# hidasib/GRU4Rec

Measured on AMD Instinct MI355X. Metric: mini-batches/sec (gru4rec.py:661), RSC15-shaped batch=128 n_sample=2048 BPR-max, higher is better.
Workload: dtype f32

## Files before the change

### gru4rec_amd/csrc/g4r_eval_kernels.cuh

```cuda
#pragma once
#include "g4r_step_kernels.cuh"

#define SC_BM 128
#define SC_KC 128

template <int TN, bool COUNT = false>
__global__ __launch_bounds__(256) void k_score_all(const DevModel* __restrict__ mp, const float* h, int mrows, const int* item_idx,
                                                   long long n_sel, float* out, long long ldo, int apply_act,
                                                   int* cnt = nullptr, long long col_begin = 0, const int* tie_col = nullptr,
                                                   unsigned tie_ctr = 0) {
    extern __shared__ __attribute__((aligned(16))) float smem[];
    const DevModel& m = *mp;
    const int tid = threadIdx.x, lane = tid & 63, wid = tid >> 6, li = lane & 15, lg = lane >> 4;
    const int D = m.Dtop;
    const int ldk = SC_KC + 2;
    float* sA = smem;
    float* sB = sA + SC_BM * ldk;
    int* sItem = reinterpret_cast<int*>(sB + TN * ldk);
    const long long n0 = (long long)blockIdx.x * TN;
    const int rbase = blockIdx.y * SC_BM;
    if (tid < TN) {
        const long long n = n0 + tid;
        int item = -1;
        if (n < n_sel) item = item_idx ? item_idx[n] : (int)n;
// ... 182 lines not shown

__global__ void k_selftest_mfma32(const float* A, const float* Bm, float* C, int K) {
    const int lane = threadIdx.x & 63, l32 = lane & 31, lh = lane >> 5;
    f32x16 acc;
    for (int j = 0; j < 16; ++j) acc[j] = 0.f;
    for (int k = 0; k < K; k += 2) acc = mfma32(A[l32 * K + k + lh], Bm[(k + lh) * 32 + l32], acc);
    for (int r = 0; r < 16; ++r) C[(8 * (r >> 2) + 4 * lh + (r & 3)) * 32 + l32] = acc[r];
}

template __global__ void k_sparse_update<1, false>(const DevModel*, StepState*, int);
template __global__ void k_sparse_update<1, true>(const DevModel*, StepState*, int);
template __global__ void k_sparse_update<2, false>(const DevModel*, StepState*, int);
template __global__ void k_sparse_update<2, true>(const DevModel*, StepState*, int);
template __global__ void k_sparse_update_generic<1>(const DevModel*, StepState*, int, int);
template __global__ void k_sparse_update_generic<2>(const DevModel*, StepState*, int, int);
template __global__ void k_loss_rows<false, 0, 1>(const DevModel*, StepState*);
template __global__ void k_loss_rows<false, 0, 4>(const DevModel*, StepState*);
template __global__ void k_loss_rows<false, 1, 1>(const DevModel*, StepState*);
template __global__ void k_loss_rows<false, 1, 4>(const DevModel*, StepState*);
template __global__ void k_loss_rows<false, 2, 1>(const DevModel*, StepState*);
template __global__ void k_loss_rows<false, 2, 4>(const DevModel*, StepState*);
template __global__ void k_loss_rows<false, 3, 1>(const DevModel*, StepState*);
template __global__ void k_loss_rows<false, 3, 4>(const DevModel*, StepState*);
template __global__ void k_loss_rows<true, 0, 4>(const DevModel*, StepState*);
template __global__ void k_loss_rows<true, 1, 4>(const DevModel*, StepState*);
template __global__ void k_loss_rows<true, 2, 4>(const DevModel*, StepState*);
template __global__ void k_loss_rows<true, 3, 4>(const DevModel*, StepState*);
template __global__ void k_sparse_update<4, false>(const DevModel*, StepState*, int);
template __global__ void k_sparse_update<4, true>(const DevModel*, StepState*, int);
template __global__ void k_sparse_update_generic<4>(const DevModel*, StepState*, int, int);
template __global__ void k_update<1, 32, false>(const DevModel*, StepState*, const DenseTile*, int, int);
template __global__ void k_update<1, 32, true>(const DevModel*, StepState*, const DenseTile*, int, int);
template __global__ void k_update<2, 32, false>(const DevModel*, StepState*, const DenseTile*, int, int);
template __global__ void k_update<2, 32, true>(const DevModel*, StepState*, const DenseTile*, int, int);
template __global__ void k_dense_grad<32>(const DevModel*, StepState*, const DenseTile*);
template __global__ void k_score_fwd<GT_BN, GT_BK>(const DevModel*, StepState*);
template __global__ void k_score_fwd<32, 64>(const DevModel*, StepState*);
template __global__ void k_score_fwd<64, 32, T2_BK>(const DevModel*, StepState*);
template __global__ void k_score_fwd<64, 32, 3>(const DevModel*, StepState*);
template __global__ void k_score_bwd<32, GT_BK>(const DevModel*, StepState*, int, int, int, int);
template __global__ void k_score_bwd<64, 64>(const DevModel*, StepState*, int, int, int, int);
template __global__ void k_gru_p1<GT_BN, P1_BK>(const DevModel*, StepState*, int, int, int, GruFwdPredict);
// ... 8 lines not shown
```

### gru4rec_amd/csrc/g4r_host_create.hpp

```cpp

int g4r_device_count(void) {
    int n = 0;
    if (hipGetDeviceCount(&n) != hipSuccess) return 0;
    return n;
}
const char* g4r_last_error(void) { return g_err.c_str(); }
#ifndef G4R_HIPCC_VERSION
#define G4R_HIPCC_VERSION "unknown"
#endif
const char* g4r_version(void) { return "gru4rec_hip 0.4 (gfx950; hipcc " G4R_HIPCC_VERSION "; isa-audited)"; }
int g4r_sizeof_config(void) { return (int)sizeof(g4r_config); }

static int build_lean_args(g4r_model* m) {
    DevModel& d = m->dm;
    const StepKernels& k = m->kern;
    const int L = d.n_layers;
    std::vector<LeanV> av(L); std::vector<LeanH> ah(L); std::vector<LeanDa> aa(L); std::vector<LeanDy> ay(L);
    const bool constrained = d.embed_mode == G4R_EMBED_CONSTRAINED;
    bool any_layer = false;
    for (int l = 0; l < L; ++l) {
        if (k.fwd[l] != FWD_LEAN) continue;
        any_layer = true;
        LeanV& v = av[l]; memset(&v, 0, sizeof(v));
        v.Wx = d.dense_p + d.offWx[l]; v.Wrz = d.dense_p + d.offWrz[l]; v.Bh = d.dense_p + d.offBh[l];
// ... 59 lines not shown
        m->h_leanU.own_on = d.own_pos ? 1 : 0;
        const bool pays = cdiv(d.R, LOSS_NW) > G4R_OWN_WINDOW_MINWG;
        m->own_window = d.own_pos && d.R <= G4R_OWN_WINDOW_MAXR && (m->sw.owner_window > 0 || (m->sw.owner_window < 0 && pays));
        HIPCHK(hipMemcpyAsync(m->d_tiles16, tiles.data(), tiles.size() * sizeof(DenseTile), hipMemcpyHostToDevice, m->stream));
        HIPCHK(hipStreamSynchronize(m->stream));
    }
    HIPCHK(hipStreamSynchronize(m->stream));
    return 0;
}

static KernelSwitches read_switches(const g4r_config& cfg) {
    KernelSwitches w;
    w.no_lean = getenv("G4R_NO_LEAN") != nullptr; w.no_mt = getenv("G4R_NO_MT") != nullptr; w.no_bmt = getenv("G4R_NO_BMT") != nullptr;
    w.no_merge = getenv("G4R_NO_MERGE") != nullptr; w.owner_scan_in_update = env_int("G4R_OWNER_SCAN", 0) != 0;
    w.owner_window = env_int("G4R_OWNER_WINDOW", -1);
    w.score_b_split = env_int("G4R_SCORE_B_SPLIT", 1) != 0;
    w.allow_lean_update = env_int("G4R_LEAN_UPDATE", 1) != 0; w.defer = env_int("G4R_DEFER", cfg.defer_updates) != 0;
    w.p2_geo = env_int("G4R_P2_GEO", -1); w.ba_geo = env_int("G4R_BA_GEO", -1);
    w.wide2 = env_int("G4R_WIDE2", -1); w.p1_ks = env_int("G4R_P1_KS", 128); w.bb_ks = env_int("G4R_BB_KS", 0);
    const char* skip = getenv("G4R_SKIP_KN");
    w.skip_kn = skip ? strtoull(skip, nullptr, 0) : 0ull;
    return w;
}

int g4r_create(const g4r_config* cfg, g4r_model** out) {
    if (!cfg || !out) return fail("null argument");
    if (cfg->n_layers < 1 || cfg->n_layers > G4R_MAX_LAYERS) return fail("n_layers out of range");
    if (cfg->batch_size < 1 || cfg->n_items < 1) return fail("batch_size / n_items must be positive");
    for (int l = 0; l < cfg->n_layers; ++l)
        if (cfg->layers[l] % 4 != 0 || cfg->layers[l] < 4 || cfg->layers[l] > 1024)
// ... 275 lines not shown
```

### gru4rec_amd/csrc/g4r_host_debug.hpp

```cpp
int g4r_get_debug(g4r_model* m, const char* name, float* host, int64_t count) {
    if (!m || !name || !host) return fail("null argument");
    HIPCHK(hipSetDevice(m->cfg.device));
    DevModel& d = m->dm;
    const StepKernels& k = m->kern;
    std::string s(name);
    const float* p = nullptr; int64_t n = 0;
    int l = 0;
    if (!s.empty() && isdigit((unsigned char)s.back())) { l = s.back() - '0'; s.pop_back(); }
    if (l >= d.n_layers) return fail("layer out of range");
    const int64_t bd = (int64_t)d.B * d.D[l];
    if (s == "scores") { p = d.Sc; n = (int64_t)d.B * d.ldSc; }
    else if (s == "dSx") { p = d.dSx + (size_t)((m->gstep - 1) & d.defer_mask) * (size_t)d.dSx_stride; n = (int64_t)d.B * d.Ein; }
    else if (s == "dSy") { p = d.dSy + (size_t)((m->gstep - 1) & d.defer_mask) * (size_t)d.dSy_stride; n = (int64_t)d.ldSc * d.Dtop; }
    else if (s == "dSBy") { p = d.dSBy + (size_t)((m->gstep - 1) & d.defer_mask) * (size_t)d.dSBy_stride; n = d.ldSc; }
    else if (s == "defer_stats") {
        if (count < 4) return fail("count");
        double rows = 0, bias = 0;
        if (m->defer_on) {
            std::vector<unsigned> st(2048);
            HIPCHK(hipStreamSynchronize(m->stream));
            HIPCHK(hipMemcpy(st.data(), d.dstat, st.size() * sizeof(unsigned), hipMemcpyDeviceToHost));
            for (size_t i = 0; i < st.size(); i += 2) { rows += st[i]; bias += st[i + 1]; }
        }
        host[0] = (float)rows; host[1] = (float)bias; host[2] = m->defer_on ? 1.f : 0.f; host[3] = (float)(d.defer_mask + 1);
// ... 25 lines not shown
    else if (s == "hd") { p = d.hd[l]; n = bd; }
    else if (s == "r") { p = d.r[l]; n = bd; }
    else if (s == "z") { p = d.z[l]; n = bd; }
    else if (s == "c") { p = d.c[l]; n = bd; }
    else if (s == "Hr") { p = d.Hr[l]; n = bd; }
    else if (s == "dV") { p = d.dV[l]; n = bd * 3; }
    else if (s == "dyl") { p = d.dyl[l]; n = bd; }
    else if (s == "Hprev") { p = d.H[l][(m->gstep + 1) & 1]; n = bd; }
    else if (s == "occ_idx") { p = (const float*)d.occ_idx; n = d.R; }
    else if (s == "own_pos") {
        if (!d.own_pos) return fail("no owner table (k_update_l not chosen, or G4R_OWNER_SCAN=1)");
        p = (const float*)(d.own_pos + (m->own_window ? (size_t)m->own_last * d.R * 16 : (size_t)0)); n = 16 * (int64_t)d.R;
    }
    else if (s == "own_pos_ring") { if (!d.own_pos) return fail("no owner table (k_update_l not chosen, or G4R_OWNER_SCAN=1)"); p = (const float*)d.own_pos; n = (int64_t)G4R_OWN_SLOTS * 16 * d.R; }
    else if (s == "owner_window") { if (count < 1) return fail("count"); host[0] = (m->own_window && k.update == UP_LEAN) ? 1.f : 0.f; return 0; }
#if !defined(G4R_CLK_TRACE)
    else if (s == "dbgclk" || s == "dbgtile") return fail("in-kernel traces need a library built with G4R_BUILD_CLK=1 (python -m gru4rec_amd.build --force) and G4R_CLK=1 at run time");
#endif
    else if (s == "dbgclk") { if (!d.dbgclk) return fail("G4R_CLK not set"); p = (const float*)d.dbgclk; n = 2 * (64 + 8 * (int64_t)d.R); }
    else if (s == "dbgtile") { if (!d.dbgtile) return fail("G4R_CLK not set"); p = (const float*)d.dbgtile; n = 2 * 8 * (int64_t)8192; }
    else if (s == "ntiles") { if (count < 1) return fail("count"); host[0] = (float)m->ntiles; return 0; }
    else if (s == "ldSc") { if (count < 1) return fail("count"); host[0] = (float)d.ldSc; return 0; }
    else if (s == "wide_mask") {
        if (count < 1) return fail("count");
        int mk = k.wide_dense ? 16 : 0;
        for (int l = 0; l < d.n_layers; ++l) mk |= k.wg[l].use;
        host[0] = (float)mk; return 0;
    }
    else if (s == "deep_geo") {
        if (count < 1) return fail("count");
// ... 48 lines not shown
}

int g4r_debug_loss_rows(g4r_model* m, float* scores, int64_t count, int32_t M, float* lossrow) {
    if (!m || !scores || !lossrow) return fail("null argument");
    DevModel& d = m->dm;
    if (count != (int64_t)d.B * d.ldSc) return fail("size mismatch for the score rows: expected " + std::to_string((int64_t)d.B * d.ldSc));
    if (M < 1 || M > d.B) return fail("M outside [1, batch_size]");
    HIPCHK(hipSetDevice(m->cfg.device));
    HIPCHK(hipStreamSynchronize(m->stream));
    StepState saved, mine;
    HIPCHK(hipMemcpy(&saved, (const void*)d.st, sizeof(saved), hipMemcpyDeviceToHost));
    HIPCHK(hipMemcpy((void*)d.Sc, scores, (size_t)count * sizeof(float), hipMemcpyHostToDevice));
    mine = saved;
    mine.M_b = M;
    HIPCHK(hipMemcpy((void*)d.st, &mine, sizeof(mine), hipMemcpyHostToDevice));
    launch_loss_rows(m, dim3(d.B), false, nullptr, nullptr);
    hipError_t e = hipGetLastError();
    if (e == hipSuccess) e = hipStreamSynchronize(m->stream);
    const hipError_t r = hipMemcpy((void*)d.st, &saved, sizeof(saved), hipMemcpyHostToDevice);
    if (e != hipSuccess) return fail(std::string("k_loss_rows: ") + hipGetErrorString(e));
    if (r != hipSuccess) return fail(std::string("step state: ") + hipGetErrorString(r));
    HIPCHK(hipMemcpy(scores, (const void*)d.Sc, (size_t)count * sizeof(float), hipMemcpyDeviceToHost));
    HIPCHK(hipMemcpy(lossrow, (const void*)d.lossrow, (size_t)d.B * sizeof(float), hipMemcpyDeviceToHost));
    return 0;
}

int g4r_debug_gumbel(g4r_model* m, uint64_t seed, uint32_t row_id, uint32_t step, const int32_t* items, int64_t n, float* out) {
    if (!m || !items || !out) return fail("null argument");
    if (n < 1) return fail("n must be positive");
    for (int64_t p = 0; p < n; ++p)
        if (items[p] < 0) return fail("item index out of range");
// ... 135 lines not shown
```

### gru4rec_amd/csrc/g4r_host_model.hpp

```cpp
static thread_local std::string g_err;
static int fail(const std::string& s) { g_err = s; return -1; }
void g4r_set_error(const char* fmt, ...) {
    char buf[1024];
    va_list ap;
    va_start(ap, fmt);
    vsnprintf(buf, sizeof(buf), fmt, ap);
    va_end(ap);
    g_err = buf;
}
#define HIPCHK(x)                                                                                        \
    do {                                                                                                 \
        hipError_t e_ = (x);                                                                             \
        if (e_ != hipSuccess)                                                                            \
            return fail(std::string(#x) + ": " + hipGetErrorString(e_) + " @" + std::to_string(__LINE__)); \
    } while (0)
#define NCCLCHK(x)                                                                                         \
    do {                                                                                                   \
        ncclResult_t e_ = (x);                                                                             \
        if (e_ != ncclSuccess)                                                                             \
            return fail(std::string(#x) + ": " + ncclGetErrorString(e_) + " @" + std::to_string(__LINE__)); \
    } while (0)

enum { KN_GRU_P1 = 0, KN_GRU_P2, KN_SCORE_FWD, KN_LOSS, KN_SCORE_BWD, KN_BWD_PRE, KN_BWD_A, KN_BWD_B, KN_DENSE, KN_ALLREDUCE,
       KN_DENSE_APPLY, KN_SPARSE, KN_UPDATE, KN_BWD_FUSED, KN_FWD_FUSED, KN_GATE, KN_FLUSH, KN_SCAN, KN_FINISH, KN_GRU_V, KN_GRU_H, KN_GRU_DA, KN_GRU_DY, KN_OWNER_WINDOW, KN_COUNT };
static const char* KN_NAMES[KN_COUNT] = {"k_gru_p1", "k_gru_p2", "k_score_fwd", "k_loss_rows", "k_score_bwd", "k_gru_bwd_pre",
                                         "k_gru_bwd_a", "k_gru_bwd_b", "k_dense_grad", "rccl_allreduce", "k_dense_apply",
                                         "k_sparse_update", "k_update", "k_gru_bwd", "k_gru_fwd", "k_gru_gate", "k_sparse_flush", "k_defer_scan", "k_finish_rows", "k_gru_v", "k_gru_h", "k_gru_da", "k_gru_dy", "k_owner_window"};

struct EvRec { int kn; hipEvent_t a, b; };

struct KernelSwitches {
    bool no_lean = false;
    bool no_mt = false, no_bmt = false;
    bool no_merge = false;
    bool allow_lean_update = true;
    bool score_b_split = true;
    bool owner_scan_in_update = false;
    int owner_window = -1;
    bool defer = false;
    int p2_geo = -1, ba_geo = -1;
    int wide2 = -1, p1_ks = 128, bb_ks = 0;
    unsigned long long skip_kn = 0;
};
enum GruFwdKind { FWD_LEAN = 0 , FWD_FUSED = 1 , FWD_P1S = 2 ,
                  FWD_P1_N64 = 3, FWD_P1_N32 = 4 };
enum GruBwdKind { BWD_LEAN = 0 , BWD_FUSED = 1 , BWD_ONEHOT = 2, BWD_BW = 3, BWD_B = 4 };
enum ScoreFwdKind { SF_LEAN = 0 , SF_MT = 1 , SF_T3 = 2, SF_T2 = 3, SF_K64 = 4, SF_K128 = 5  };
enum ScoreBwdKind { SB_LEAN = 0 , SB_BMT = 1 , SB_BWD2 = 2 , SB_W = 3, SB_N = 4  };
enum UpdateKind { UP_LEAN = 0 , UP_MERGED = 1 , UP_SPLIT = 2 };
struct WideGeo { int use = 0, ny = 1, nh = 1, kys = 0, khs = 0, bbn = 1, bbk = 0; };
struct StepKernels {
    int fwd[G4R_MAX_LAYERS], bwd[G4R_MAX_LAYERS];
    int p2_deep[G4R_MAX_LAYERS], ba_deep[G4R_MAX_LAYERS];
    WideGeo wg[G4R_MAX_LAYERS];
    int score_fwd;
    int loss_spec, loss_long, loss_quads;
    int score_bwd;
    int score_a_host;
    int kch, ksplit;
    int bmt_slabs;
    int nblkA, nblkB, ndtA, ndtB, nrtB;
    int update;
    int chunks;
    int wide_dense;
    int finish_rows;
};

template <class T>
struct DevBuf {
    T* p = nullptr;
    int64_t cap = 0;
    int reserve(g4r_model* m, int64_t n);
};

struct g4r_model {
    g4r_config cfg;
    DevModel dm;
// ... 320 lines not shown
            const double waste = (std::ceil(rounds) - rounds) / std::ceil(rounds) + 1e-3 * std::abs(ks - 17);
            if (waste < best) { best = waste; k.kch = kch; }
        }
    }
    k.ksplit = cdiv(d.ldSc, k.kch);
    const int TB = wide ? 64 : 32;
    k.ndtA = cdiv(Dt + 1, TB); k.nblkA = cdiv(d.ldSc, TB) * k.ndtA;
    k.ndtB = cdiv(Dt, TB); k.nrtB = cdiv(B, TB); k.nblkB = k.ksplit * k.nrtB * k.ndtB;
    const int w = std::max(Dt, d.Ein);
    k.chunks = w <= 256 ? 1 : (w <= 512 ? 2 : 4);
    const bool dy0_parts = (k.wg[0].use & 8) != 0;
    const bool merged = !d.generic && !sw.no_merge && k.chunks <= 2 && !k.wide_dense;
    const bool lean_u = !sw.no_lean && sw.allow_lean_update && merged && d.apply_dense_inplace && B <= 128 && k.chunks == 1 && !defer_on && d.xmode == 0 &&
                        !d.touched && !dy0_parts && d.R < 65536 && cdiv(d.R, 8) < 65536 && dense_tiles(d, 16, 64).size() < 65536;
    k.update = lean_u ? UP_LEAN : merged ? UP_MERGED : UP_SPLIT;
    k.finish_rows = dy0_parts && !k.wide_dense;
    return k;
}
static int sync_dm(g4r_model* m) {
    HIPCHK(hipMemcpyAsync(m->d_dm, &m->dm, sizeof(DevModel), hipMemcpyHostToDevice, m->stream));
    HIPCHK(hipStreamSynchronize(m->stream));
    return 0;
}
```

### gru4rec_amd/csrc/g4r_host_step.hpp

```cpp
static void launch_loss_rows(g4r_model* m, dim3 grid, bool timed, hipEvent_t ev_a, hipEvent_t ev_b) {
    const StepKernels& k = m->kern;
    const DevModel* dmp = (const DevModel*)m->d_dm;
    StepState* stp = (StepState*)m->dm.st;
#define G4R_LK_LOSS1(kern)                                                                                            \
    do {                                                                                                              \
        if (timed) hipExtLaunchKernelGGL(kern, grid, dim3(LOSS_T), m->smem_loss, m->stream, ev_a, ev_b, 0, dmp, stp); \
        else hipLaunchKernelGGL(kern, grid, dim3(LOSS_T), m->smem_loss, m->stream, dmp, stp);                         \
    } while (0)
#define G4R_LK_LOSS(L, V)                                                      \
    do {                                                                       \
        if (k.loss_spec == 1) G4R_LK_LOSS1((k_loss_rows<L, 1, V>));            \
        else if (k.loss_spec == 2) G4R_LK_LOSS1((k_loss_rows<L, 2, V>));       \
        else if (k.loss_spec == 3) G4R_LK_LOSS1((k_loss_rows<L, 3, V>));       \
        else G4R_LK_LOSS1((k_loss_rows<L, 0, V>));                             \
    } while (0)
    if (k.loss_long) G4R_LK_LOSS(true, 4);
    else { if (k.loss_quads) G4R_LK_LOSS(false, 4); else G4R_LK_LOSS(false, 1); }
#undef G4R_LK_LOSS
#undef G4R_LK_LOSS1
}

static int launch_step(g4r_model* m, std::vector<EvRec>* recs, int part = 0, int slot = 0) {
    DevModel& d = m->dm;
    const StepKernels& k = m->kern;
    const int L = d.n_layers, B = d.B;
    hipStream_t s = m->stream;
    GruFwdPredict nopa = {};
    size_t evi = 0;
    hipEvent_t cur_a = nullptr, cur_b = nullptr;
    static const bool trace = getenv("G4R_TRACE") != nullptr;
    int trace_kn = -1;
    auto begin = [&](int kn) {
        trace_kn = kn;
        if (trace) { fprintf(stderr, "[g4r] launch %s\n", KN_NAMES[kn]); fflush(stderr); }
        if (!recs) return;
        while (m->evs.size() < evi + 2) { hipEvent_t e; (void)hipEventCreate(&e); m->evs.push_back(e); }
        EvRec r = {kn, m->evs[evi], m->evs[evi + 1]};
// ... 77 lines not shown
                (const float*)d.Wy, (const float*)d.By, (float*)d.Sc, dimsA, dimsB);
        break;
    }
    case SF_MT: LK(k_score_mt_4s, dim3(cdiv(B, 64) * cdiv(d.ldSc, 272)), dim3(256), SMEM_MT_4S, s, (const int*)d.cur_col, (const int*)(d.cur_in + 2 * B),
                   (const float*)d.hd[L - 1], (const float*)d.Wy, (const float*)d.zrow, dmp, (unsigned)d.Dtop | ((unsigned)cdiv(B, 64) << 16),
                   (unsigned)d.N, (unsigned)d.ldSc, (unsigned)B); break;
    case SF_T3: LK(k_score_fwd_t3, dim3(cdiv(d.ldSc, 64), cdiv(B, 64)), dim3(GT_NTH), SMEM_SF3, s, dmp, stp); break;
    case SF_T2: LK(k_score_fwd_t2, dim3(cdiv(d.ldSc, 64), cdiv(B, 64)), dim3(GT_NTH), SMEM_SF2, s, dmp, stp); break;
    case SF_K64: LK(k_score_fwd_k64, dim3(cdiv(d.ldSc, SFW_BN), cdiv(B, SF_BM)), dim3(GT_NTH), SMEM_SF64, s, dmp, stp); break;
    default: LK(k_score_fwd_k128, dim3(cdiv(d.ldSc, GT_BN), cdiv(B, SF_BM)), dim3(GT_NTH), SMEM_SF, s, dmp, stp); break;
    }
    end();
    begin(KN_LOSS);
    {
        const int nown = std::min(cdiv(d.R, LOSS_NW), std::max(2 * m->n_cu - B, 32));
        const dim3 gloss(B + (merged && k.update == UP_LEAN && d.own_pos && !m->own_window ? nown : 0));
        if (!(m->sw.skip_kn && ((m->sw.skip_kn >> KN_LOSS) & 1ull))) launch_loss_rows(m, gloss, recs != nullptr, cur_a, cur_b);
    }
    end();
    begin(KN_SCORE_BWD);
    switch (k.score_bwd) {
    case SB_LEAN: {
        const LeanB& q = m->h_leanB;
#define G4R_LK_SB(RA, NWG) LK(k_score_b<RA>, dim3(NWG), dim3(512), 0, s, (const LeanB*)m->d_leanB, (const int*)(d.cur_in + 2 * B), (const int*)d.cur_col,   \
           (const float*)d.Sc, (const float*)d.hd[L - 1], (const float*)d.Wy, (float*)d.accWy, (unsigned)d.Dtop | ((unsigned)B << 16), (unsigned)d.N | ((unsigned)d.ldSc << 16))
        if (a_hosted) G4R_LK_SB(false, d.ksplit * q.nrb * q.ndb);
        else G4R_LK_SB(true, q.nA + d.ksplit * q.nrb * q.ndb);
#undef G4R_LK_SB
        break;
    }
    case SB_BMT: {
        const int ntile = d.ldSc / BMT_WA * (d.Dtop / 32);
// ... 195 lines not shown
}
static int ensure_graph(g4r_model* m) {
    if (m->gexec) return 0;
    const bool dist = !m->dm.apply_dense_inplace && !local_staged(m);
    const bool rccl_in_graph = dist && (!m->p2p_ready || (m->exact && m->comm_ready));
    if (dist) {
        if (!m->p2p_ready) NCCLCHK(ncclAllReduce(m->dm.dense_g, m->dm.dense_g, m->dm.dense_count, ncclFloat, ncclSum, m->comm, m->stream));
        if (m->exact && m->comm_ready)
            NCCLCHK(ncclAllGather((const float*)m->dm.xbase + (size_t)m->cfg.rank * (size_t)m->dm.xstride, (float*)m->dm.xbase, (size_t)m->dm.xstride,
                                  ncclFloat, m->comm, m->stream));
        HIPCHK(hipStreamSynchronize(m->stream));
    }
    hipGraph_t graph = nullptr;
    HIPCHK(hipStreamBeginCapture(m->stream, rccl_in_graph ? hipStreamCaptureModeRelaxed : hipStreamCaptureModeThreadLocal));
    int rc = 0;
    for (int i = 0; i < G4R_GRAPH_STEPS && !rc; ++i) rc = launch_step(m, nullptr, 0, i);
    hipError_t e = hipStreamEndCapture(m->stream, &graph);
    if (rc || e != hipSuccess || !graph) {
        if (graph) (void)hipGraphDestroy(graph);
        (void)hipGetLastError();
        if (!rc) fail(std::string("graph capture: ") + hipGetErrorString(e));
        return -1;
    }
    e = hipGraphInstantiate(&m->gexec, graph, nullptr, nullptr, 0);
    (void)hipGraphDestroy(graph);
    if (e != hipSuccess) { m->gexec = nullptr; (void)hipGetLastError(); return fail(std::string("graph instantiate: ") + hipGetErrorString(e)); }
    m->graph_steps = G4R_GRAPH_STEPS;
    if (!dist) {
        hipGraph_t g2 = nullptr;
        if (hipStreamBeginCapture(m->stream, hipStreamCaptureModeThreadLocal) == hipSuccess) {
            int rc2 = 0;
            for (int i = 0; i < G4R_GRAPH_STEPS_SMALL && !rc2; ++i) rc2 = launch_step(m, nullptr, 0, i);
            hipError_t e2 = hipStreamEndCapture(m->stream, &g2);
            if (!rc2 && e2 == hipSuccess && g2 && hipGraphInstantiate(&m->gexec_small, g2, nullptr, nullptr, 0) != hipSuccess) m->gexec_small = nullptr;
            if (g2) (void)hipGraphDestroy(g2);
            (void)hipGetLastError();
        }
    }
    return 0;
}
static int ensure_head_graph(g4r_model* m);
static int ensure_step_graph(g4r_model* m, bool* whole) {
    if (m->dm.apply_dense_inplace) { *whole = true; return ensure_graph(m); }
    if (dist_graph_wanted(m)) {
        if (ensure_graph(m) == 0) { *whole = true; return 0; }
        m->dist_graph_failed = true;
        fprintf(stderr, "[g4r] RCCL all-reduce could not be captured into the step graph (%s); launching it eagerly\n", g_err.c_str());
// ... 43 lines not shown
            if (refill_store(m)) return -1;
            hipLaunchKernelGGL(k_restage_inputs, dim3(1), dim3(512), 0, m->stream, (const DevModel*)m->d_dm, (StepState*)m->dm.st);
        }
        const bool devsync = m->sync_every_dev > 0 && m->comm_ready;
        if (devsync && m->since_sync >= m->sync_every_dev) {
            if (sync_dense_enqueue(m)) return -1;
            ++m->n_dev_syncs;
        }
        int64_t run = tend - t;
        if (devsync) run = std::min<int64_t>(run, m->sync_every_dev - m->since_sync);
        if (ci < m->compact_steps.size()) run = std::min(run, m->compact_steps[ci] - t);
        if (m->dm.ns > 0 && !m->store_frozen) run = std::min<int64_t>(run, m->gl - (m->gstep % m->gl));
        if (run <= 0) return fail("internal: empty run");
        int64_t done = 0;
        const bool own_win = m->own_window && m->kern.update == UP_LEAN && !(m->profiling && m->profile_split);
        auto window_open = [&](int64_t nw) -> int {
            if (own_win && !((m->sw.skip_kn >> KN_OWNER_WINDOW) & 1ull)) {
                const DevModel& d = m->dm;
                const bool timed = m->profiling;
                if (timed) for (auto& e : m->ev_ow) if (!e) (void)hipEventCreate(&e);
                const dim3 gw((unsigned)(nw * cdiv(2 * d.B, OW_NW)));
                const size_t lds = (size_t)(((d.R + 3) & ~3) + 16 * OW_NW) * sizeof(int);
                if (timed) hipExtLaunchKernelGGL(k_owner_window, gw, dim3(OW_T), lds, m->stream, m->ev_ow[0], m->ev_ow[1], 0, (const DevModel*)m->d_dm, (long long)(t + done), (long long)(m->gstep + done), (int)nw);
                else hipLaunchKernelGGL(k_owner_window, gw, dim3(OW_T), lds, m->stream, (const DevModel*)m->d_dm, (long long)(t + done), (long long)(m->gstep + done), (int)nw);
                HIPCHK(hipGetLastError());
            }
            if (!m->defer_on) return 0;
            wguard.open = true;
            const dim3 gs(cdiv(nw * m->dm.R, 256));
            if (m->profiling) (void)hipEventRecord(m->ev_df[0], m->stream);
            hipLaunchKernelGGL(k_defer_scan, gs, dim3(256), 0, m->stream, (const DevModel*)m->d_dm, (long long)(t + done), (long long)(m->gstep + done), (int)nw, 0);
            hipLaunchKernelGGL(k_defer_scan, gs, dim3(256), 0, m->stream, (const DevModel*)m->d_dm, (long long)(t + done), (long long)(m->gstep + done), (int)nw, 1);
            if (m->profiling) (void)hipEventRecord(m->ev_df[1], m->stream);
            return 0;
        };
        auto window_close = [&](int64_t nw, int64_t first) -> int {
            if (own_win) {
// ... 8 lines not shown
            if (m->profiling) (void)hipEventRecord(m->ev_df[2], m->stream);
            hipLaunchKernelGGL(k_sparse_flush, dim3(cdiv(nw * m->dm.dRcap, SP_WAVES * FL_NR)), dim3(SP_WAVES * 64), 0, m->stream, (const DevModel*)m->d_dm, (long long)(m->gstep + first), (int)nw);
            if (m->profiling) {
                (void)hipEventRecord(m->ev_df[3], m->stream);
                HIPCHK(hipStreamSynchronize(m->stream));
                float ms = 0.f;
                if (hipEventElapsedTime(&ms, m->ev_df[0], m->ev_df[1]) == hipSuccess) { m->kn_ms[KN_SCAN] += ms; m->kn_n[KN_SCAN]++; }
                if (hipEventElapsedTime(&ms, m->ev_df[2], m->ev_df[3]) == hipSuccess) { m->kn_ms[KN_FLUSH] += ms; m->kn_n[KN_FLUSH]++; }
            }
            wguard.open = false;
            return 0;
        };
        if (use_graph && run >= G4R_GRAPH_STEPS_SMALL) {
            if (ensure_graph(m)) return -1;
            for (; done + m->graph_steps <= run; done += m->graph_steps) {
                if (window_open(m->graph_steps)) return -1;
                HIPCHK(hipGraphLaunch(m->gexec, m->stream));
                if (window_close(m->graph_steps, done)) return -1;
            }
            if (m->gexec_small)
                for (; done + G4R_GRAPH_STEPS_SMALL <= run; done += G4R_GRAPH_STEPS_SMALL) {
                    if (window_open(G4R_GRAPH_STEPS_SMALL)) return -1;
                    HIPCHK(hipGraphLaunch(m->gexec_small, m->stream));
                    if (window_close(G4R_GRAPH_STEPS_SMALL, done)) return -1;
                }
        }
        int64_t win_first = -1, win_n = 0;
        for (; done < run; ++done) {
            if ((m->defer_on || own_win) && win_n == 0) {
                win_n = std::min<int64_t>(G4R_DEFER_SLOTS, run - done); win_first = done;
                if (window_open(win_n)) return -1;
            }
            const int slot = win_n > 0 ? (int)(done - win_first) : 0;
            if (m->profiling) {
                recs.clear();
                if (launch_step(m, &recs, 0, slot)) return -1;
                HIPCHK(hipStreamSynchronize(m->stream));
                for (auto& r : recs) {
                    float ms = 0.f;
                    if (hipEventElapsedTime(&ms, r.a, r.b) == hipSuccess) { m->kn_ms[r.kn] += ms; m->kn_n[r.kn]++; }
                }
            } else if (m->cfg.use_graph && !m->dm.apply_dense_inplace && !getenv("G4R_TRACE")) {
                if (ensure_head_graph(m)) return -1;
                HIPCHK(hipGraphLaunch(m->gexec_head, m->stream));
                if (launch_step(m, nullptr, 2)) return -1;
            } else if (launch_step(m, nullptr, 0, slot)) return -1;
            if (win_n > 0 && done + 1 == win_first + win_n) {
                if (window_close(win_n, win_first)) return -1;
                win_n = 0;
            }
        }
        t += run;
        m->gstep += run;
        m->since_sync += run;
    }
    HIPCHK(hipStreamSynchronize(m->stream));
    if (m->p2p_ready) {
        unsigned late = 0;
        HIPCHK(hipMemcpy(&late, m->p2p_round + m->p2p_nblk, sizeof(late), hipMemcpyDeviceToHost));
        if (late) return fail("p2p all-reduce: a peer did not publish its gradients within G4R_P2P_TIMEOUT_MS (dead rank?)");
    }
// ... 122 lines not shown
```

### gru4rec_amd/csrc/g4r_loss_kernel.cuh

```cuda
#pragma once
#ifndef LOSS_T
#define LOSS_T 1024
#endif
#define LOSS_NW (LOSS_T / 64)
template <int NV, bool MAX>
__device__ __forceinline__ void block_reduce(float (&v)[NV], float* red) {
    const int lane = threadIdx.x & 63, w = threadIdx.x >> 6;
#pragma unroll
    for (int q = 0; q < NV; ++q) v[q] = MAX ? wave_max(v[q]) : wave_sum(v[q]);
    if (lane == 0) {
#pragma unroll
        for (int q = 0; q < NV; ++q) red[q * LOSS_NW + w] = v[q];
    }
    __syncthreads();
#pragma unroll
    for (int q = 0; q < NV; ++q) {
        float a = red[q * LOSS_NW];
#pragma unroll
        for (int u = 1; u < LOSS_NW; ++u) a = MAX ? fmaxf(a, red[q * LOSS_NW + u]) : a + red[q * LOSS_NW + u];
        v[q] = a;
    }
}

__device__ __forceinline__ float softplusf_(float x) {
// ... 48 lines not shown
                at += __popcll(mk[e] & below);
                cnt += __popcll(mk[e]);
            }
#pragma unroll
            for (int e = 0; e < 4; ++e) {
                if ((mk[e] >> lane) & 1ull) {
                    if ((unsigned)at < (unsigned)G4R_OWN_INLINE) pos[1 + at] = j0 + e;
                    ++at;
                }
            }
        }
    }
    if (lane == 0) pos[0] = min(cnt, G4R_OWN_INLINE);
}

template <bool LONG_ROW, int SPEC, int V>
__global__ __launch_bounds__(LOSS_T) void k_loss_rows(const DevModel* __restrict__ mp, StepState* st) {
    const DevModel& m = *mp;
    extern __shared__ __attribute__((aligned(16))) float smem[];
    const int tid = threadIdx.x;
    const int B = m.B, N = m.N, i = blockIdx.x;
    const int fact = SPEC == 1 || SPEC == 3 ? (int)G4R_ACT_ELU : (SPEC == 2 ? (int)G4R_ACT_SOFTMAX : m.final_act);
    const int lossk = SPEC == 1 ? (int)G4R_LOSS_BPR_MAX : (SPEC == 2 ? (int)G4R_LOSS_XE : (SPEC == 3 ? (int)G4R_LOSS_TOP1_MAX : m.loss));
    const int ldSc = m.ldSc;
    const float fp0 = m.fa_p0, fp1 = m.fa_p1, invB = m.inv_B, bpreg = m.bpreg, smooth = m.smoothing;
    GAS float* row = m.Sc + (size_t)i * ldSc;
    float* sy = smem;
    std::conditional_t<LONG_ROW, GAS float*, float*> se;
    if constexpr (LONG_ROW) se = row; else se = smem + ldSc;
    float* red = smem + (LONG_ROW ? 1 : 2) * ldSc;
    constexpr int STEP = V * LOSS_T;
    const int jt = V * tid;
    constexpr int LOSS_PRE = (V == 4) ? 2 : 4;
#if defined(G4R_CLK_TRACE)
    struct Span { GAS long long* p; __device__ ~Span() { if (p) p[1] = wall_clock64(); } } span_{(m.dbgtile && tid == 0 && i < 532) ? m.dbgtile + 8 * (size_t)(7168 + i) : nullptr};
    if (span_.p) span_.p[0] = wall_clock64();
#endif
    const StepCtx c = load_ctx(st);
    if (i >= B) {
        const unsigned nown = gridDim.x - B, R = m.R;
        for (unsigned k = (threadIdx.x >> 6) * nown + (unsigned)(i - B); k < R; k += LOSS_NW * nown) owner_prescan(m, k);
        return;
    }
    float pre_s[LOSS_PRE][V];
#pragma unroll
    for (int q = 0; q < LOSS_PRE; ++q) vld<V>(pre_s[q], row + min(jt + q * STEP, ldSc - V));
    const int M = c.M;
    if (i >= M) return;
    const bool fsm = (fact == G4R_ACT_SOFTMAX), fsl = (fact == G4R_ACT_SOFTMAX_LOGIT);
    const float n_out = (float)(M + (N - B));
    auto active = [&](int j) { return j < N && (j < M || j >= B); };
    auto grp_fast = [&](int j0) { return (j0 >= B && j0 + V <= N) || (j0 + V <= G4R_MUT_FAST_M(M) && (i < j0 || i >= j0 + V)); };
    using Fast = std::true_type;
    using Slow = std::false_type;
// ... 280 lines not shown
```

### gru4rec_amd/csrc/g4r_update_kernels.cuh

```cuda
#pragma once
__global__ __launch_bounds__(256) void k_onehot_step(const DevModel* __restrict__ mp, StepState* st) {
    const DevModel& m = *mp;
    const StepCtx c = load_ctx(st);
    const int W = m.Ein, nc4 = W >> 2;
    const long long q = (long long)blockIdx.x * 256 + threadIdx.x;
    const int row = (int)(q / nc4), c4 = (int)(q % nc4);
    if (row >= c.M) return;
    const int item = m.occ_idx[row];
    if (item < 0) return;
    const float lr = m.lr;
    const float4 g = ld4(m.dV[0] + (size_t)row * W + 4 * c4);
    const float4 a = ld4(m.accE + (size_t)item * W + 4 * c4);
    const int cnt = m.occ_fl[4 * ((size_t)m.n_items + item) + 2];
    const float4 an = make_float4(a.x + g.x * g.x, a.y + g.y * g.y, a.z + g.z * g.z, a.w + g.w * g.w);
    if (!m.generic && cnt == 1) st4(m.accE + (size_t)item * W + 4 * c4, an);
    else st4(m.dAx + (size_t)row * W + 4 * c4, an);
    if (m.generic) { st4(G4R_DSX(m, c.g) + (size_t)row * W + 4 * c4, g); return; }
    st4(G4R_DSX(m, c.g) + (size_t)row * W + 4 * c4, make_float4(lr * g.x * frsq(an.x + G4R_EPS_ADAGRAD), lr * g.y * frsq(an.y + G4R_EPS_ADAGRAD),
                                                         lr * g.z * frsq(an.z + G4R_EPS_ADAGRAD), lr * g.w * frsq(an.w + G4R_EPS_ADAGRAD)));
}

struct DenseTile {
    GP(const float) X0; GP(const float) X1; GP(const float) dV;
    long long base;
// ... 504 lines not shown
__global__ __launch_bounds__(256) void k_defer_scan(const DevModel* __restrict__ mp, long long t0, long long g0, int n, int pass) {
    const DevModel& m = *mp;
    const long long idx = (long long)blockIdx.x * 256 + threadIdx.x;
    const int R = m.R, s = (int)(idx / R), k = (int)(idx - (long long)s * R);
    if (s >= n) return;
    int table;
    const int item = defer_item(m, t0 + s, g0 + s, k, table);
    const size_t slot = G4R_SLOT(m, g0 + s) * (size_t)m.dRcap + k;
    if (item < 0) { if (pass) m.dcand[slot] = 0; return; }
    GAS int* lu = m.last_use + (size_t)table * m.n_items + item;
    if (pass == 0) atomicMax((int*)lu, (int)(g0 + s));
    else m.dcand[slot] = (*lu == (int)(g0 + s)) ? 1 : 0;
}
#define OW_T 1024
#define OW_NW (OW_T / 64)
static_assert(G4R_OWN_INLINE + 1 == 16, "an owner-table row is 16 ints: the count and G4R_OWN_INLINE positions");
static_assert(((size_t)G4R_OWN_WINDOW_MAXR + 16 * OW_NW) * sizeof(int) <= 65536, "k_owner_window: the longest list and the waves' position rows share one workgroup's 64 KB of LDS");
__global__ __launch_bounds__(OW_T) void k_owner_window(const DevModel* __restrict__ mp, long long t0, long long g0, int nw) {
    const DevModel& m = *mp;
    extern __shared__ __attribute__((aligned(16))) int sid[];
    const int R = m.R, B = m.B, Rp = (R + 3) & ~3;
    const int gps = (2 * B + OW_NW - 1) / OW_NW;
    const int s = (int)blockIdx.x / gps, q = (int)blockIdx.x - s * gps;
#if defined(G4R_CLK_TRACE)
    struct Span { GAS long long* p; __device__ ~Span() { if (p) p[1] = wall_clock64(); } } span_{(m.dbgtile && threadIdx.x == 0 && blockIdx.x < 400) ? m.dbgtile + 8 * (size_t)(7700 + blockIdx.x) : nullptr};
    if (span_.p) span_.p[0] = wall_clock64();
#endif
    if (s >= nw) return;
    for (int k = threadIdx.x; k < Rp; k += OW_T) {
        int table;
        sid[k] = k < R ? defer_item(m, t0 + s, G4R_MUT_WIN_G(g0, s), k, table) : -1;
    }
    __syncthreads();
    const int lane = threadIdx.x & 63, wid = threadIdx.x >> 6;
    const int p = q * OW_NW + wid;
    if (p >= 2 * B) return;
    const int item = sid[p];
    if (item < 0) return;
    const bool constrained = m.embed_mode == G4R_EMBED_CONSTRAINED;
    const int ta = (constrained || p < B) ? 0 : B, tb = (!constrained && p < B) ? B : R;
    int* spos = sid + Rp + 16 * wid;
    const unsigned long long below = (1ull << lane) - 1ull;
    int cnt = 0, last = p;
    for (int base0 = ta & ~3; base0 < tb; base0 += 1024) {
        int4 vv[4];
#pragma unroll
// ... 31 lines not shown
                    ++at;
                }
                cnt += __popcll(mk[e]);
            }
        }
    }
    if (cnt < 2) return;
    GAS int* pos = m.own_pos + ((size_t)s * (size_t)R + (size_t)last) * 16;
    if (cnt - 1 > G4R_OWN_INLINE) {
        if (lane == 0) pos[0] = -1;
        return;
    }
    __builtin_amdgcn_fence(__ATOMIC_ACQ_REL, "wavefront");
    if (lane < cnt - 1) pos[1 + lane] = spos[lane];
    if (lane == 0) pos[0] = cnt - 1;
}
#define FL_NR 4
__global__ __launch_bounds__(SP_WAVES * 64) void k_sparse_flush(const DevModel* __restrict__ mp, long long g0, int n) {
    const DevModel& m = *mp;
    const int lane = threadIdx.x & 63, wid = threadIdx.x >> 6;
    const long long e0 = ((long long)blockIdx.x * SP_WAVES + wid) * FL_NR;
    const int Rc = m.dRcap, s = (int)(e0 / Rc), k0 = (int)(e0 - (long long)s * Rc);
    if (s >= n) return;
    const size_t slot = G4R_SLOT(m, g0 + s) * (size_t)Rc + k0;
    int it[FL_NR];
#pragma unroll
    for (int u = 0; u < FL_NR; ++u) it[u] = m.dlist[slot + u];
    if (lane < FL_NR) { m.dcand[slot + lane] = 0; m.dlist[slot + lane] = -1; }
    const int B = m.B;
    const bool sep = m.embed_mode != G4R_EMBED_CONSTRAINED;
// ... 384 lines not shown
```

Baseline: 27000.

## Optionally host owner-window scan inside loss-rows launch or graph head

Moves the owner-window scan into a shared device function, so extra workgroups of the k_loss_rows launch can run it (mode 1), or a k_owner_window_a kernel can run it at the head of the captured graph (mode 2). The goal is to drop a separate host-side kernel launch per graph window. The id-gathering loop is also rewritten to issue four independent loads per thread through a direct index-address helper instead of calling defer_item per element. The new modes are off by default (owner_window_host=0), so by default only the reworked load loop changes.

```diff
diff --git a/gru4rec_amd/csrc/g4r_eval_kernels.cuh b/gru4rec_amd/csrc/g4r_eval_kernels.cuh
--- a/gru4rec_amd/csrc/g4r_eval_kernels.cuh
+++ b/gru4rec_amd/csrc/g4r_eval_kernels.cuh
@@ -220,18 +220,18 @@
 template __global__ void k_sparse_update<2, true>(const DevModel*, StepState*, int);
 template __global__ void k_sparse_update_generic<1>(const DevModel*, StepState*, int, int);
 template __global__ void k_sparse_update_generic<2>(const DevModel*, StepState*, int, int);
-template __global__ void k_loss_rows<false, 0, 1>(const DevModel*, StepState*);
-template __global__ void k_loss_rows<false, 0, 4>(const DevModel*, StepState*);
-template __global__ void k_loss_rows<false, 1, 1>(const DevModel*, StepState*);
-template __global__ void k_loss_rows<false, 1, 4>(const DevModel*, StepState*);
-template __global__ void k_loss_rows<false, 2, 1>(const DevModel*, StepState*);
-template __global__ void k_loss_rows<false, 2, 4>(const DevModel*, StepState*);
-template __global__ void k_loss_rows<false, 3, 1>(const DevModel*, StepState*);
-template __global__ void k_loss_rows<false, 3, 4>(const DevModel*, StepState*);
-template __global__ void k_loss_rows<true, 0, 4>(const DevModel*, StepState*);
-template __global__ void k_loss_rows<true, 1, 4>(const DevModel*, StepState*);
-template __global__ void k_loss_rows<true, 2, 4>(const DevModel*, StepState*);
-template __global__ void k_loss_rows<true, 3, 4>(const DevModel*, StepState*);
+template __global__ void k_loss_rows<false, 0, 1>(const DevModel*, StepState*, int);
+template __global__ void k_loss_rows<false, 0, 4>(const DevModel*, StepState*, int);
+template __global__ void k_loss_rows<false, 1, 1>(const DevModel*, StepState*, int);
+template __global__ void k_loss_rows<false, 1, 4>(const DevModel*, StepState*, int);
+template __global__ void k_loss_rows<false, 2, 1>(const DevModel*, StepState*, int);
+template __global__ void k_loss_rows<false, 2, 4>(const DevModel*, StepState*, int);
+template __global__ void k_loss_rows<false, 3, 1>(const DevModel*, StepState*, int);
+template __global__ void k_loss_rows<false, 3, 4>(const DevModel*, StepState*, int);
+template __global__ void k_loss_rows<true, 0, 4>(const DevModel*, StepState*, int);
+template __global__ void k_loss_rows<true, 1, 4>(const DevModel*, StepState*, int);
+template __global__ void k_loss_rows<true, 2, 4>(const DevModel*, StepState*, int);
+template __global__ void k_loss_rows<true, 3, 4>(const DevModel*, StepState*, int);
 template __global__ void k_sparse_update<4, false>(const DevModel*, StepState*, int);
 template __global__ void k_sparse_update<4, true>(const DevModel*, StepState*, int);
 template __global__ void k_sparse_update_generic<4>(const DevModel*, StepState*, int, int);
diff --git a/gru4rec_amd/csrc/g4r_host_create.hpp b/gru4rec_amd/csrc/g4r_host_create.hpp
--- a/gru4rec_amd/csrc/g4r_host_create.hpp
+++ b/gru4rec_amd/csrc/g4r_host_create.hpp
@@ -97,6 +97,7 @@
     w.no_lean = getenv("G4R_NO_LEAN") != nullptr; w.no_mt = getenv("G4R_NO_MT") != nullptr; w.no_bmt = getenv("G4R_NO_BMT") != nullptr;
     w.no_merge = getenv("G4R_NO_MERGE") != nullptr; w.owner_scan_in_update = env_int("G4R_OWNER_SCAN", 0) != 0;
     w.owner_window = env_int("G4R_OWNER_WINDOW", -1);
+    w.owner_window_host = env_int("G4R_OWNER_WINDOW_HOST", w.owner_window_host);
     w.score_b_split = env_int("G4R_SCORE_B_SPLIT", 1) != 0;
     w.allow_lean_update = env_int("G4R_LEAN_UPDATE", 1) != 0; w.defer = env_int("G4R_DEFER", cfg.defer_updates) != 0;
     w.p2_geo = env_int("G4R_P2_GEO", -1); w.ba_geo = env_int("G4R_BA_GEO", -1);
diff --git a/gru4rec_amd/csrc/g4r_host_debug.hpp b/gru4rec_amd/csrc/g4r_host_debug.hpp
--- a/gru4rec_amd/csrc/g4r_host_debug.hpp
+++ b/gru4rec_amd/csrc/g4r_host_debug.hpp
@@ -63,6 +63,7 @@
     }
     else if (s == "own_pos_ring") { if (!d.own_pos) return fail("no owner table (k_update_l not chosen, or G4R_OWNER_SCAN=1)"); p = (const float*)d.own_pos; n = (int64_t)G4R_OWN_SLOTS * 16 * d.R; }
     else if (s == "owner_window") { if (count < 1) return fail("count"); host[0] = (m->own_window && k.update == UP_LEAN) ? 1.f : 0.f; return 0; }
+    else if (s == "owner_window_host") { if (count < 1) return fail("count"); host[0] = (m->own_window && k.update == UP_LEAN) ? (float)k.own_host : 0.f; return 0; }
 #if !defined(G4R_CLK_TRACE)
     else if (s == "dbgclk" || s == "dbgtile") return fail("in-kernel traces need a library built with G4R_BUILD_CLK=1 (python -m gru4rec_amd.build --force) and G4R_CLK=1 at run time");
 #endif
@@ -141,7 +142,7 @@
     mine = saved;
     mine.M_b = M;
     HIPCHK(hipMemcpy((void*)d.st, &mine, sizeof(mine), hipMemcpyHostToDevice));
-    launch_loss_rows(m, dim3(d.B), false, nullptr, nullptr);
+    launch_loss_rows(m, dim3(d.B), m->smem_loss, 0, false, nullptr, nullptr);
     hipError_t e = hipGetLastError();
     if (e == hipSuccess) e = hipStreamSynchronize(m->stream);
     const hipError_t r = hipMemcpy((void*)d.st, &saved, sizeof(saved), hipMemcpyHostToDevice);
diff --git a/gru4rec_amd/csrc/g4r_host_model.hpp b/gru4rec_amd/csrc/g4r_host_model.hpp
--- a/gru4rec_amd/csrc/g4r_host_model.hpp
+++ b/gru4rec_amd/csrc/g4r_host_model.hpp
@@ -37,6 +37,7 @@
     bool score_b_split = true;
     bool owner_scan_in_update = false;
     int owner_window = -1;
+    int owner_window_host = 0;
     bool defer = false;
     int p2_geo = -1, ba_geo = -1;
     int wide2 = -1, p1_ks = 128, bb_ks = 0;
@@ -61,6 +62,7 @@
     int bmt_slabs;
     int nblkA, nblkB, ndtA, ndtB, nrtB;
     int update;
+    int own_host;
     int chunks;
     int wide_dense;
     int finish_rows;
@@ -411,6 +413,7 @@
     const bool lean_u = !sw.no_lean && sw.allow_lean_update && merged && d.apply_dense_inplace && B <= 128 && k.chunks == 1 && !defer_on && d.xmode == 0 &&
                         !d.touched && !dy0_parts && d.R < 65536 && cdiv(d.R, 8) < 65536 && dense_tiles(d, 16, 64).size() < 65536;
     k.update = lean_u ? UP_LEAN : merged ? UP_MERGED : UP_SPLIT;
+    k.own_host = k.update == UP_LEAN ? std::min(std::max(sw.owner_window_host, 0), 2) : 0;
     k.finish_rows = dy0_parts && !k.wide_dense;
     return k;
 }
diff --git a/gru4rec_amd/csrc/g4r_host_step.hpp b/gru4rec_amd/csrc/g4r_host_step.hpp
--- a/gru4rec_amd/csrc/g4r_host_step.hpp
+++ b/gru4rec_amd/csrc/g4r_host_step.hpp
@@ -1,11 +1,11 @@
-static void launch_loss_rows(g4r_model* m, dim3 grid, bool timed, hipEvent_t ev_a, hipEvent_t ev_b) {
+static void launch_loss_rows(g4r_model* m, dim3 grid, size_t lds, int nwin, bool timed, hipEvent_t ev_a, hipEvent_t ev_b) {
     const StepKernels& k = m->kern;
     const DevModel* dmp = (const DevModel*)m->d_dm;
     StepState* stp = (StepState*)m->dm.st;
 #define G4R_LK_LOSS1(kern)                                                                                            \
     do {                                                                                                              \
-        if (timed) hipExtLaunchKernelGGL(kern, grid, dim3(LOSS_T), m->smem_loss, m->stream, ev_a, ev_b, 0, dmp, stp); \
-        else hipLaunchKernelGGL(kern, grid, dim3(LOSS_T), m->smem_loss, m->stream, dmp, stp);                         \
+        if (timed) hipExtLaunchKernelGGL(kern, grid, dim3(LOSS_T), lds, m->stream, ev_a, ev_b, 0, dmp, stp, nwin);    \
+        else hipLaunchKernelGGL(kern, grid, dim3(LOSS_T), lds, m->stream, dmp, stp, nwin);                            \
     } while (0)
 #define G4R_LK_LOSS(L, V)                                                      \
     do {                                                                       \
@@ -20,7 +20,12 @@
 #undef G4R_LK_LOSS1
 }
 
-static int launch_step(g4r_model* m, std::vector<EvRec>* recs, int part = 0, int slot = 0) {
+static bool hosts_window(const g4r_model* m, bool recs, int part) {
+    return m->kern.own_host == 1 && m->own_window && m->kern.update == UP_LEAN && part == 0 && !recs && !((m->sw.skip_kn >> KN_LOSS) & 1ull);
+}
+static size_t owner_window_lds(const DevModel& d) { return (size_t)(((d.R + 3) & ~3) + 16 * OW_NW) * sizeof(int); }
+
+static int launch_step(g4r_model* m, std::vector<EvRec>* recs, int part = 0, int slot = 0, int nw = 0) {
     DevModel& d = m->dm;
     const StepKernels& k = m->kern;
     const int L = d.n_layers, B = d.B;
@@ -128,8 +133,11 @@
     begin(KN_LOSS);
     {
         const int nown = std::min(cdiv(d.R, LOSS_NW), std::max(2 * m->n_cu - B, 32));
-        const dim3 gloss(B + (merged && k.update == UP_LEAN && d.own_pos && !m->own_window ? nown : 0));
-        if (!(m->sw.skip_kn && ((m->sw.skip_kn >> KN_LOSS) & 1ull))) launch_loss_rows(m, gloss, recs != nullptr, cur_a, cur_b);
+        const bool hosted = slot == 0 && nw > 0 && hosts_window(m, recs != nullptr, part) && !((m->sw.skip_kn >> KN_OWNER_WINDOW) & 1ull);
+        const int nwin = hosted ? nw * cdiv(2 * B, OW_NW) : 0;
+        const dim3 gloss(B + nwin + (merged && k.update == UP_LEAN && d.own_pos && !m->own_window ? nown : 0));
+        const size_t lds = hosted ? std::max(m->smem_loss, owner_window_lds(d)) : m->smem_loss;
+        if (!(m->sw.skip_kn && ((m->sw.skip_kn >> KN_LOSS) & 1ull))) launch_loss_rows(m, gloss, lds, hosted ? nw : 0, recs != nullptr, cur_a, cur_b);
     }
     end();
     begin(KN_SCORE_BWD);
@@ -355,7 +363,13 @@
     hipGraph_t graph = nullptr;
     HIPCHK(hipStreamBeginCapture(m->stream, rccl_in_graph ? hipStreamCaptureModeRelaxed : hipStreamCaptureModeThreadLocal));
     int rc = 0;
-    for (int i = 0; i < G4R_GRAPH_STEPS && !rc; ++i) rc = launch_step(m, nullptr, 0, i);
+    const bool own_head = m->kern.own_host == 2 && m->own_window && m->kern.update == UP_LEAN && !((m->sw.skip_kn >> KN_OWNER_WINDOW) & 1ull);
+    auto window_head = [&](int nw) {
+        if (own_head) hipLaunchKernelGGL(k_owner_window_a, dim3((unsigned)(nw * cdiv(2 * m->dm.B, OW_NW))), dim3(OW_T), owner_window_lds(m->dm), m->stream,
+                                         (const DevModel*)m->d_dm, (const StepState*)m->dm.st, nw);
+    };
+    window_head(G4R_GRAPH_STEPS);
+    for (int i = 0; i < G4R_GRAPH_STEPS && !rc; ++i) rc = launch_step(m, nullptr, 0, i, G4R_GRAPH_STEPS);
     hipError_t e = hipStreamEndCapture(m->stream, &graph);
     if (rc || e != hipSuccess || !graph) {
         if (graph) (void)hipGraphDestroy(graph);
@@ -371,7 +385,8 @@
         hipGraph_t g2 = nullptr;
         if (hipStreamBeginCapture(m->stream, hipStreamCaptureModeThreadLocal) == hipSuccess) {
             int rc2 = 0;
-            for (int i = 0; i < G4R_GRAPH_STEPS_SMALL && !rc2; ++i) rc2 = launch_step(m, nullptr, 0, i);
+            window_head(G4R_GRAPH_STEPS_SMALL);
+            for (int i = 0; i < G4R_GRAPH_STEPS_SMALL && !rc2; ++i) rc2 = launch_step(m, nullptr, 0, i, G4R_GRAPH_STEPS_SMALL);
             hipError_t e2 = hipStreamEndCapture(m->stream, &g2);
             if (!rc2 && e2 == hipSuccess && g2 && hipGraphInstantiate(&m->gexec_small, g2, nullptr, nullptr, 0) != hipSuccess) m->gexec_small = nullptr;
             if (g2) (void)hipGraphDestroy(g2);
@@ -445,13 +460,14 @@
         if (run <= 0) return fail("internal: empty run");
         int64_t done = 0;
         const bool own_win = m->own_window && m->kern.update == UP_LEAN && !(m->profiling && m->profile_split);
-        auto window_open = [&](int64_t nw) -> int {
-            if (own_win && !((m->sw.skip_kn >> KN_OWNER_WINDOW) & 1ull)) {
+        auto window_open = [&](int64_t nw, bool graph) -> int {
+            const bool elsewhere = graph ? (m->kern.own_host == 2 || hosts_window(m, false, 0)) : hosts_window(m, m->profiling, 0);
+            if (own_win && !elsewhere && !((m->sw.skip_kn >> KN_OWNER_WINDOW) & 1ull)) {
                 const DevModel& d = m->dm;
                 const bool timed = m->profiling;
                 if (timed) for (auto& e : m->ev_ow) if (!e) (void)hipEventCreate(&e);
                 const dim3 gw((unsigned)(nw * cdiv(2 * d.B, OW_NW)));
-                const size_t lds = (size_t)(((d.R + 3) & ~3) + 16 * OW_NW) * sizeof(int);
+                const size_t lds = owner_window_lds(d);
                 if (timed) hipExtLaunchKernelGGL(k_owner_window, gw, dim3(OW_T), lds, m->stream, m->ev_ow[0], m->ev_ow[1], 0, (const DevModel*)m->d_dm, (long long)(t + done), (long long)(m->gstep + done), (int)nw);
                 else hipLaunchKernelGGL(k_owner_window, gw, dim3(OW_T), lds, m->stream, (const DevModel*)m->d_dm, (long long)(t + done), (long long)(m->gstep + done), (int)nw);
                 HIPCHK(hipGetLastError());
@@ -490,13 +506,13 @@
         if (use_graph && run >= G4R_GRAPH_STEPS_SMALL) {
             if (ensure_graph(m)) return -1;
             for (; done + m->graph_steps <= run; done += m->graph_steps) {
-                if (window_open(m->graph_steps)) return -1;
+                if (window_open(m->graph_steps, true)) return -1;
                 HIPCHK(hipGraphLaunch(m->gexec, m->stream));
                 if (window_close(m->graph_steps, done)) return -1;
             }
             if (m->gexec_small)
                 for (; done + G4R_GRAPH_STEPS_SMALL <= run; done += G4R_GRAPH_STEPS_SMALL) {
-                    if (window_open(G4R_GRAPH_STEPS_SMALL)) return -1;
+                    if (window_open(G4R_GRAPH_STEPS_SMALL, true)) return -1;
                     HIPCHK(hipGraphLaunch(m->gexec_small, m->stream));
                     if (window_close(G4R_GRAPH_STEPS_SMALL, done)) return -1;
                 }
@@ -505,12 +521,12 @@
         for (; done < run; ++done) {
             if ((m->defer_on || own_win) && win_n == 0) {
                 win_n = std::min<int64_t>(G4R_DEFER_SLOTS, run - done); win_first = done;
-                if (window_open(win_n)) return -1;
+                if (window_open(win_n, false)) return -1;
             }
             const int slot = win_n > 0 ? (int)(done - win_first) : 0;
             if (m->profiling) {
                 recs.clear();
-                if (launch_step(m, &recs, 0, slot)) return -1;
+                if (launch_step(m, &recs, 0, slot, (int)win_n)) return -1;
                 HIPCHK(hipStreamSynchronize(m->stream));
                 for (auto& r : recs) {
                     float ms = 0.f;
@@ -520,7 +536,7 @@
                 if (ensure_head_graph(m)) return -1;
                 HIPCHK(hipGraphLaunch(m->gexec_head, m->stream));
                 if (launch_step(m, nullptr, 2)) return -1;
-            } else if (launch_step(m, nullptr, 0, slot)) return -1;
+            } else if (launch_step(m, nullptr, 0, slot, (int)win_n)) return -1;
             if (win_n > 0 && done + 1 == win_first + win_n) {
                 if (window_close(win_n, win_first)) return -1;
                 win_n = 0;
diff --git a/gru4rec_amd/csrc/g4r_loss_kernel.cuh b/gru4rec_amd/csrc/g4r_loss_kernel.cuh
--- a/gru4rec_amd/csrc/g4r_loss_kernel.cuh
+++ b/gru4rec_amd/csrc/g4r_loss_kernel.cuh
@@ -86,8 +86,9 @@
     if (lane == 0) pos[0] = min(cnt, G4R_OWN_INLINE);
 }
 
+__device__ __forceinline__ void owner_window_scan(const DevModel& m, long long t0, long long g0, int nw, int wg, int* sid);
 template <bool LONG_ROW, int SPEC, int V>
-__global__ __launch_bounds__(LOSS_T) void k_loss_rows(const DevModel* __restrict__ mp, StepState* st) {
+__global__ __launch_bounds__(LOSS_T) void k_loss_rows(const DevModel* __restrict__ mp, StepState* st, int nwin) {
     const DevModel& m = *mp;
     extern __shared__ __attribute__((aligned(16))) float smem[];
     const int tid = threadIdx.x;
@@ -110,6 +111,7 @@
 #endif
     const StepCtx c = load_ctx(st);
     if (i >= B) {
+        if (nwin > 0) { owner_window_scan(m, c.t, c.g, nwin, i - B, reinterpret_cast<int*>(smem)); return; }
         const unsigned nown = gridDim.x - B, R = m.R;
         for (unsigned k = (threadIdx.x >> 6) * nown + (unsigned)(i - B); k < R; k += LOSS_NW * nown) owner_prescan(m, k);
         return;
diff --git a/gru4rec_amd/csrc/g4r_update_kernels.cuh b/gru4rec_amd/csrc/g4r_update_kernels.cuh
--- a/gru4rec_amd/csrc/g4r_update_kernels.cuh
+++ b/gru4rec_amd/csrc/g4r_update_kernels.cuh
@@ -542,22 +542,52 @@
 }
 #define OW_T 1024
 #define OW_NW (OW_T / 64)
+static_assert(OW_T == LOSS_T, "the window scan also runs in workgroups of the k_loss_rows launch (g4r_loss_kernel.cuh)");
 static_assert(G4R_OWN_INLINE + 1 == 16, "an owner-table row is 16 ints: the count and G4R_OWN_INLINE positions");
 static_assert(((size_t)G4R_OWN_WINDOW_MAXR + 16 * OW_NW) * sizeof(int) <= 65536, "k_owner_window: the longest list and the waves' position rows share one workgroup's 64 KB of LDS");
-__global__ __launch_bounds__(OW_T) void k_owner_window(const DevModel* __restrict__ mp, long long t0, long long g0, int nw) {
-    const DevModel& m = *mp;
-    extern __shared__ __attribute__((aligned(16))) int sid[];
+struct OwnerIds {
+    unsigned long long ax, ay, as;
+    int B;
+    __device__ __forceinline__ OwnerIds(const DevModel& m, long long t, long long g) : B(m.B) {
+        const long long tB = t * (long long)m.B;
+        const long long srow = (long long)(m.gl > 0 ? g % m.gl : 0) * m.ns;
+        ax = (unsigned long long)m.in_idx + 4ull * (unsigned long long)tB;
+        ay = (unsigned long long)m.out_idx + 4ull * (unsigned long long)(tB - m.B);
+        as = (unsigned long long)m.ST + 4ull * (unsigned long long)(srow - 2 * m.B);
+    }
+    __device__ __forceinline__ int at(int k, int& need) const {
+        const bool x = k < B, y = k < 2 * B;
+        need = x ? k : (y ? k - B : 0);
+        const unsigned long long a = (x ? ax : (y ? ay : as)) + 4ull * (unsigned)k;
+        return *(const GAS int*)a;
+    }
+};
+#define OW_STAGE 4
+__device__ __forceinline__ void owner_window_scan(const DevModel& m, long long t0, long long g0, int nw, int wg, int* sid) {
     const int R = m.R, B = m.B, Rp = (R + 3) & ~3;
     const int gps = (2 * B + OW_NW - 1) / OW_NW;
-    const int s = (int)blockIdx.x / gps, q = (int)blockIdx.x - s * gps;
+    const int s = wg / gps, q = wg - s * gps;
 #if defined(G4R_CLK_TRACE)
-    struct Span { GAS long long* p; __device__ ~Span() { if (p) p[1] = wall_clock64(); } } span_{(m.dbgtile && threadIdx.x == 0 && blockIdx.x < 400) ? m.dbgtile + 8 * (size_t)(7700 + blockIdx.x) : nullptr};
+    struct Span { GAS long long* p; __device__ ~Span() { if (p) p[1] = wall_clock64(); } } span_{(m.dbgtile && threadIdx.x == 0 && wg < 400) ? m.dbgtile + 8 * (size_t)(7700 + wg) : nullptr};
     if (span_.p) span_.p[0] = wall_clock64();
 #endif
     if (s >= nw) return;
-    for (int k = threadIdx.x; k < Rp; k += OW_T) {
-        int table;
-        sid[k] = k < R ? defer_item(m, t0 + s, G4R_MUT_WIN_G(g0, s), k, table) : -1;
+    {
+        const long long t = t0 + s, g = G4R_MUT_WIN_G(g0, s);
+        const int M = m.Mplan[t];
+        const OwnerIds ids(m, t, g);
+        for (int k0 = threadIdx.x; k0 < Rp; k0 += OW_STAGE * OW_T) {
+            int v[OW_STAGE], need[OW_STAGE];
+#pragma unroll
+            for (int u = 0; u < OW_STAGE; ++u) v[u] = ids.at(min(k0 + u * OW_T, R - 1), need[u]);
+            asm volatile("" : "+v"(v[0]), "+v"(v[1]), "+v"(v[2]), "+v"(v[3]));
+            static_assert(OW_STAGE == 4, "the line above names four values");
+#pragma unroll
+            for (int u = 0; u < OW_STAGE; ++u) {
+                const int k = k0 + u * OW_T;
+                if (k < Rp) sid[k] = (k < R && need[u] < M) ? v[u] : -1;
+            }
+        }
     }
     __syncthreads();
     const int lane = threadIdx.x & 63, wid = threadIdx.x >> 6;
@@ -619,6 +649,15 @@
     __builtin_amdgcn_fence(__ATOMIC_ACQ_REL, "wavefront");
     if (lane < cnt - 1) pos[1 + lane] = spos[lane];
     if (lane == 0) pos[0] = cnt - 1;
+}
+__global__ __launch_bounds__(OW_T) void k_owner_window(const DevModel* __restrict__ mp, long long t0, long long g0, int nw) {
+    extern __shared__ __attribute__((aligned(16))) int sid[];
+    owner_window_scan(*mp, t0, g0, nw, (int)blockIdx.x, sid);
+}
+__global__ __launch_bounds__(OW_T) void k_owner_window_a(const DevModel* __restrict__ mp, const StepState* st_, int nw) {
+    extern __shared__ __attribute__((aligned(16))) int sid[];
+    const GAS StepState* st = (const GAS StepState*)st_;
+    owner_window_scan(*mp, st->t_a, st->g_a, nw, (int)blockIdx.x, sid);
 }
 #define FL_NR 4
 __global__ __launch_bounds__(SP_WAVES * 64) void k_sparse_flush(const DevModel* __restrict__ mp, long long g0, int n) {
```

Measured after the change: 27000 (median of 4 runs). About the same (-0.0%).
